# simeoncarstens/binf

Hardware: AMD Instinct MI355X
Metric: chain*leapfrog-steps/sec, 1024-d Gaussian (higher is better)
Workload: dtype f64

## Files before the change

### binf_amd/_native.py

```python
import ctypes
import linecache
import os

import torch

_HERE = os.path.dirname(os.path.abspath(__file__))
LIB_PATH = os.environ.get('BINF_LIB_OVERRIDE') or \
    os.path.join(_HERE, 'csrc', 'libbinf_hip.so')

MODE_EXACT = 0
MODE_FMA = 1
MODE_LANE_PER_CHAIN = 16
MOVE_HMC = 0
MOVE_RWMC = 1

E_ARG = -1
E_UNSUPPORTED = -2
E_ALIAS = -3


class NativeLibraryError(RuntimeError):
    """libbinf_hip.so is missing, stale or failed."""


# ... 9 lines not shown
    'binf_abi_version': (_i32, []),
    'binf_last_error': (_i32, [ctypes.c_char_p, ctypes.c_size_t]),
    'binf_hmc_sample_gauss_f64': (_i32, [_vp, _vp, _vp, _vp, _vp, _vp, _vp, _vp,
                                         _f64, _vp, _i64, _i64, _i32, _f64,
                                         _f64, _i32, _f64, _f64, _i32, _vp]),
    'binf_hmc_sample_n_gauss_f64': (_i32, [_vp, _vp, _vp, _vp, _vp, _vp, _vp,
                                           _vp, _vp, _f64, _vp, _i64, _i64,
                                           _i32, _i32, _i32, _f64, _f64, _i32,
                                           _f64, _f64, _i32, _vp]),
    'binf_hmc_gauss_waves_per_chain': (_i32, [_i64, _i64]),
    'binf_hmc_sample_gauss_big_workspace_bytes': (_i64, [_i64, _i64]),
    'binf_hmc_sample_gauss_big_f64': (_i32, [_vp, _vp, _vp, _vp, _vp, _vp, _vp, _vp,
                                             _f64, _vp, _i64, _i64, _i32, _f64,
                                             _f64, _i32, _f64, _f64, _i32, _vp,
                                             _i64, _vp]),
    'binf_hmc_sample_gauss_big_rng_f64': (_i32, [_vp, _vp, _vp, _vp, _vp, _vp, _f64, _vp,
                                                 _i64, _i64, _i32, _f64, _f64, _i32,
                                                 _f64, _f64, _i32, ctypes.c_uint64,
                                                 ctypes.c_uint64, _i64, _vp, _i64, _vp]),
    'binf_hmc_sample_n_gauss_big_workspace_bytes': (_i64, [_i64, _i64]),
    'binf_hmc_sample_n_gauss_big_f64': (_i32, [_vp, _vp, _vp, _vp, _vp, _vp, _vp, _vp, _vp,
                                               _f64, _vp, _i64, _i64, _i32, _i32, _i32, _f64,
                                               _f64, _i32, _f64, _f64, _i32, _vp, _i64, _vp]),
    'binf_hmc_sample_n_gauss_big_rng_f64': (_i32, [_vp, _vp, _vp, _vp, _vp, _vp, _vp, _f64, _vp,
                                                   _i64, _i64, _i32, _i32, _i32, _f64, _f64,
                                                   _i32, _f64, _f64, _i32, _u64, _u64, _i64,
                                                   _vp, _i64, _vp]),
    'binf_hmc_gauss_big_rng_draws_f64': (_i32, [_vp, _vp, _i64, _i64, ctypes.c_uint64,
                                                ctypes.c_uint64, _i64, _vp]),
    'binf_hmc_sample_n_gauss_rng_f64': (_i32, [_vp, _vp, _vp, _vp, _vp, _vp, _vp,
                                               _f64, _vp, _i64, _i64, _i32, _i32,
                                               _i32, _f64, _f64, _i32, _f64, _f64,
                                               _i32, ctypes.c_uint64,
                                               ctypes.c_uint64, _i64, _vp]),
    'binf_hmc_gauss_rng_draws_f64': (_i32, [_vp, _vp, _i64, _i64, _i32,
                                            ctypes.c_uint64, ctypes.c_uint64, _i64, _vp]),
    'binf_hmc_sample_poly_f64': (_i32, [_vp, _vp, _vp, _vp, _vp, _vp, _vp, _vp,
                                        _vp, _vp, _f64, _vp, _vp, _vp, _i32,
                                        _vp, _vp, _f64, _vp, _i64, _i64, _i64,
                                        _i32, _i32, _f64, _f64, _i32, _vp]),
    'binf_clipped_exp_f64': (_i32, [_vp, _vp, _i64, _vp]),
    'binf_row_sum_f64': (_i32, [_vp, _vp, _i64, _i64, _i32, _f64, _f64, _vp]),
    'binf_hmc_energy_f64': (_i32, [_vp, _vp, _vp, _i64, _i64, _vp]),
    'binf_gamma_logp_f64': (_i32, [_vp, _f64, _f64, _vp, _i64, _vp]),
    'binf_leapfrog_kick_f64': (_i32, [_vp, _vp, _f64, _vp, _i32, _i64, _i64,
                                      _i32, _vp]),
    'binf_leapfrog_drift_f64': (_i32, [_vp, _vp, _f64, _vp, _i64, _i64, _i32,
                                       _vp]),
    'binf_leapfrog_kick_drift_f64': (_i32, [_vp, _vp, _vp, _f64, _vp, _i64, _i64,
                                            _i32, _vp]),
    'binf_gauss_grad_f64': (_i32, [_vp, _vp, _f64, _f64, _i64, _i64, _vp]),
    'binf_accept_select_f64': (_i32, [_vp, _vp, _vp, _vp, _vp, _vp, _vp, _vp, _vp,
                                      _i32, _f64, _f64, _i64, _i64, _vp]),
    'binf_row_sumsq_diff_f64': (_i32, [_vp, _vp, _vp, _vp, _i64, _i64, _f64,
                                       _vp]),
    'binf_poly_forward_f64': (_i32, [_vp, _vp, _vp, _i64, _i64, _i64, _vp]),
    'binf_predictive_density_workspace_bytes': (_i64, [_i64, _i64, _i64]),
    'binf_predictive_density_f64': (_i32, [_vp, _vp, _vp, _vp, _i64, _i64, _i64, _f64, _vp, _i64, _vp]),
    'binf_gauss_err_grad_f64': (_i32, [_vp, _vp, _f64, _vp, _vp, _i64, _i64,
                                       _vp]),
    'binf_gauss_err_logp_f64': (_i32, [_vp, _vp, _f64, _vp, _vp, _i64, _i64,
                                       _vp]),
    'binf_poly_gauss_logp_f64': (_i32, [_vp, _vp, _vp, _f64, _vp, _vp, _i64,
                                        _i64, _i64, _vp]),
    'binf_poly_gauss_logp_memo_f64': (_i32, [_vp, _vp, _vp, _f64, _vp, _vp, _vp, _vp, _vp,
                                             _i64, _i64, _i64, _vp]),
    'binf_poly_gauss_grad_workspace_bytes': (_i64, [_i64, _i64, _i64]),
    'binf_poly_gauss_grad_f64': (_i32, [_vp, _vp, _vp, _f64, _vp, _vp, _vp,
                                        _i64, _i64, _i64, _i64, _vp]),
    'binf_linear_forward_f64': (_i32, [_vp, _vp, _vp, _i64, _i64, _i64, _vp]),
    'binf_linear_gauss_logp_workspace_bytes': (_i64, [_i64, _i64, _i64]),
    'binf_linear_gauss_logp_f64': (_i32, [_vp, _vp, _vp, _f64, _vp, _vp, _vp,
                                          _i64, _i64, _i64, _i64, _vp]),
    'binf_gamma_precision_update_f64': (_i32, [_vp, _vp, _f64, _vp, _i64, _vp]),
    'binf_poly_leapfrog_workspace_bytes': (_i64, [_i64, _i64, _i64]),
    'binf_poly_leapfrog_f64': (_i32, [_vp, _vp, _vp, _vp, _f64, _vp, _vp, _i64, _i64, _i64, _i64,
                                      _f64, _vp, _i32, _i32, _vp]),
    'binf_pairdist_chi2_workspace_bytes': (_i64, [_i64, _i64, _i64]),
    'binf_pairdist_gauss_logp_f64': (_i32, [_vp, _vp, _vp, _vp, _f64, _vp, _vp, _i64,
                                            _i64, _i64, _vp, _i64, _vp]),
    'binf_pairdist_gauss_logp_memo_f64': (_i32, [_vp, _vp, _vp, _vp, _f64, _vp, _vp, _vp, _vp, _vp,
                                                 _i64, _i64, _i64, _vp, _i64, _vp]),
    'binf_pairdist_forward_f64': (_i32, [_vp, _vp, _vp, _vp, _i64, _i64, _i64,
                                         _vp]),
    'binf_pairdist_gauss_grad_f64': (_i32, [_vp, _vp, _f64, _vp, _vp, _i64,
                                            _i64, _vp]),
    'binf_pairdist_leapfrog_f64': (_i32, [_vp, _vp, _vp, _f64, _vp, _i32, _f64,
                                          _f64, _i32, _f64, _vp, _i32, _i64,
                                          _i64, _i32, _vp]),
    'binf_pairdist_hmc_energy_f64': (_i32, [_vp, _vp, _vp, _vp, _vp, _f64, _vp, _f64, _f64, _i32,
                                            ctypes.POINTER(_i32), _vp, _f64, _vp, _f64,
                                            _vp, _vp, _vp, _vp, _vp, _i64, _i64, _i64, _vp, _i64, _vp]),
    'binf_pairdist_packed_targets_bytes': (_i64, [_i64]),
    'binf_pairdist_pack_targets_f64': (_i32, [_vp, _vp, _i64, _vp]),
    'binf_pairdist_tiles_workspace_bytes': (_i64, [_i64, _i64]),
    'binf_pairdist_gauss_grad_packed_f64': (_i32, [_vp, _vp, _vp, _f64, _vp, _vp, _i64,
                                                   _i64, _vp, _i64, _vp]),
    'binf_pairdist_leapfrog_packed_f64': (_i32, [_vp, _vp, _vp, _vp, _vp, _f64, _vp, _i32, _f64,
                                                 _f64, _i32, _f64, _vp, _i32, _i64,
                                                 _i64, _i32, _vp, _i64, _vp]),
    'binf_rng_uniform_f64': (_i32, [_vp, _i64, ctypes.c_uint64, ctypes.c_uint64,
                                    _i64, _vp]),
    'binf_rng_normal_f64': (_i32, [_vp, _i64, ctypes.c_uint64, ctypes.c_uint64,
                                   _i64, _vp]),
    'binf_rng_normal_zig_uniform_f64': (_i32, [_vp, _i64, _vp, _i64, ctypes.c_uint64, ctypes.c_uint64,
                                               ctypes.c_uint64, _i64, _i64, _vp]),
# ... 320 lines not shown
def metric_comoments(x, k0, s1, s2, first):
    C, D = _cd(x)
    G = _groups(s2, C, D, *_CHOL_FACTORS)
    rc = lib().binf_metric_comoments_f64(
        dptr(x, numel=C * D, name='x'), dptr(k0, numel=G * D, name='k0'),
        dptr(s1, numel=G * D, name='s1'), dptr(s2, numel=G * D * D, name='s2'),
        int(bool(first)), C, D, G, stream_handle(x.device))
    check(rc, 'binf_metric_comoments_f64')


@_launcher
def metric_factor(s1, s2, n, C, chol, work, status=None, regularise=True):
    D = s2.shape[-1]
    G = _groups(s2, int(C), D, *_CHOL_FACTORS)
    rc = lib().binf_metric_factor_f64(
        dptr(s1, numel=G * D, name='s1'), dptr(s2, numel=G * D * D, name='s2'), int(n), int(C),
        D, G, int(bool(regularise)), dptr(chol, numel=G * D * D, name='chol'),
        dptr(work, numel=G * D * D, name='work'), dptr(status, torch.int32, G, 'status'),
        stream_handle(s2.device))
    check(rc, 'binf_metric_factor_f64')


@_launcher
def gauss_grad(x, k, x0, out=None):
    C, D = _cd(x)
    if out is None:
        out = torch.empty_like(x)
    rc = lib().binf_gauss_grad_f64(dptr(x, numel=C * D, name='x'),
                                   dptr(out, numel=C * D, name='out'),
                                   float(k), float(x0), C, D,
                                   stream_handle(x.device))
    check(rc, 'binf_gauss_grad_f64')
    return out


@_launcher
def accept_select(q_prop, q_old, e_before, e_after, u, q_out, accepted,
                  n_accepted=None, dt_chain=None, adapt=False, uprate=1.05, downrate=0.95):
    C, D = _cd(q_prop)
    n = C * D
    rc = lib().binf_accept_select_f64(
        dptr(q_prop, numel=n, name='q_prop'), dptr(q_old, numel=n, name='q_old'),
        dptr(e_before, numel=C, name='e_before'),
        dptr(e_after, numel=C, name='e_after'), dptr(u, numel=C, name='u'),
        dptr(q_out, numel=n, name='q_out'),
        dptr(accepted, torch.uint8, C, 'accepted'),
        dptr(n_accepted, torch.int64, C, 'n_accepted'),
        dptr(dt_chain, numel=C, name='dt_chain'), int(bool(adapt)),
        float(uprate), float(downrate), C, D, stream_handle(q_prop.device))
    check(rc, 'binf_accept_select_f64')


@_launcher
def clipped_exp(x):
    require_device(x, 'x')
    xc = x.contiguous()
    out = torch.empty_like(xc)
    rc = lib().binf_clipped_exp_f64(dptr(xc), dptr(out), xc.numel(),
                                    stream_handle(x.device))
    check(rc, 'binf_clipped_exp_f64')
    return out


def require_device(x, what):
    if not (isinstance(x, torch.Tensor) and x.is_cuda):
        raise TypeError('%s must be a ROCm (cuda) fp64 tensor, got %s; binf_amd '
                        'evaluates on the GPU only (no CPU path)'
                        % (what, type(x).__name__ if not isinstance(x, torch.Tensor)
                           else 'a %s tensor' % x.device.type))
    return x


def _precision_args(precision, C, device):
    if isinstance(precision, torch.Tensor):
        if precision.dim() == 0:
            return float(precision), None
        p = precision.reshape(-1)
        if p.numel() != C:
            raise ValueError('precision has %d entries for %d chains'
                             % (p.numel(), C))
        return 0.0, p.contiguous()
    return float(precision), None


@_launcher
def row_sumsq_diff(x, y, scale=1.0, weights=None):
    C, D = _cd(x)
    out = torch.empty(C, dtype=torch.float64, device=x.device)
    rc = lib().binf_row_sumsq_diff_f64(dptr(x, numel=C * D, name='x'),
                                       dptr(y, numel=D, name='y'),
                                       dptr(weights, numel=D, name='weights'),
                                       dptr(out), C, D, float(scale),
                                       stream_handle(x.device))
    check(rc, 'binf_row_sumsq_diff_f64')
    return out


@_launcher
def poly_forward(coeffs, xs):
    C, K = _cd(coeffs)
    N = xs.numel()
    out = torch.empty((C, N), dtype=torch.float64, device=coeffs.device)
    rc = lib().binf_poly_forward_f64(dptr(coeffs, numel=C * K, name='coeffs'),
                                     dptr(xs, numel=N, name='xs'), dptr(out),
                                     C, K, N, stream_handle(coeffs.device))
    check(rc, 'binf_poly_forward_f64')
# ... 1129 lines not shown
```

### binf_amd/csrc/gauss_common.hpp

```cpp
#pragma once
#include "common.hpp"

namespace binf {

struct GaussNArgs {
    const double *q0;
    const double *p0;
    const double *u;
    double *q_out;
    double *samples;
    uint8_t *accepted;
    int64_t *n_accepted;
    double *e_before;
    double *e_after;
    double *dt_chain;
    double timestep;
    double k;
    double x0;
    double uprate;
    double downrate;
    int64_t C;
    int32_t D;
    int32_t nsteps;
    int32_t H;
// ... 20 lines not shown
    int LW;
    int tneed;
    bool regular;
    int64_t blocks;
};

inline GaussPlan gauss_plan(int64_t C, int64_t D)
{
    GaussPlan p;
    p.H = pairwise_tree_height(D);
    p.LW = p.H > 3 ? p.H - 3 : 0;
    p.tneed = 1;
    p.regular = true;
    int32_t len0 = -1;
    for (int g = 0; g < (1 << p.H); ++g) {
        Leaf L = pairwise_leaf((int32_t)D, p.H, g);
        int tn = (L.len + 7) / 8;
        if (tn > p.tneed) p.tneed = tn;
        if (len0 < 0) len0 = L.len;
        if (L.len != len0 || L.depth != p.H || (L.len & 7)) p.regular = false;
    }
    if (p.LW == 0) {
        const int64_t chains_per_wave = 64 >> (3 + p.H);
        const int64_t waves = (C + chains_per_wave - 1) / chains_per_wave;
        p.blocks = (waves + 3) / 4;
    } else {
        const int64_t chains_per_block = (p.LW == 3 ? 8 : 4) >> p.LW;
        p.blocks = (C + chains_per_block - 1) / chains_per_block;
    }
    return p;
}

int gauss_split_factor(int64_t C, int32_t H, bool regular, int tneed);
hipError_t launch_gauss_split(const GaussNArgs &a, int tneed, int split, bool unit, bool fma,
                              hipStream_t st);

struct LaneSum {
    double r;
    double tail;
};

template <bool REGULAR>
__device__ inline void lane_sum_add(LaneSum &s, double v, int t, int T)
{
    if (REGULAR) {
        s.r = (t == 0) ? v : s.r + v;
    } else {
        const double n = s.r + v;
        s.r = (t == 0) ? v : ((t < T) ? n : s.r);
        s.tail = (t == T) ? v : s.tail;
    }
}

template <bool REGULAR, int LW = 0>
__device__ inline double chain_sum_finish(const LaneSum &s, int T, int rem,
                                          int lane, int H, int leafdepth,
                                          double *xch = nullptr, int wib = 0)
{
    const double r = sum8_f64(s.r);
    double res = r;
    if (!REGULAR) {
        res = (T > 0) ? r : -0.0;
        const int leafbase = lane & ~7;
#pragma unroll
        for (int i = 0; i < 7; ++i) {
            const double v = shfl_f64(s.tail, leafbase + i);
            const double n = res + v;
            res = (i < rem) ? n : res;
        }
    }
    const int hin = (LW > 0) ? 3 : H;
    for (int l = 0; l < hin; ++l) {
        const double o = xor_level_f64(res, l, lane);
        const double n = res + o;
        res = (leafdepth >= H - l) ? n : res;
    }
    if (LW > 0) {
#pragma unroll
        for (int l = 3; l < 3 + LW; ++l) {
            __syncthreads();
            if (lane == 0) xch[wib] = res;
            __syncthreads();
            const double o = xch[wib ^ (1 << (l - 3))];
            const double n = res + o;
            res = (leafdepth >= H - l) ? n : res;
        }
    }
    return 0.0 + res;
}

template <int H, int N>
__device__ inline void chain_sum_finish_fixed(double (&v)[N], int lane)
{
    static_assert(H >= 0 && H <= 3, "one-wave chains: at most 8 leaves");
#pragma unroll
    for (int i = 0; i < N; ++i) v[i] = v[i] + xor1_f64(v[i]);
#pragma unroll
    for (int i = 0; i < N; ++i) v[i] = v[i] + xor2_f64(v[i]);
#pragma unroll
    for (int i = 0; i < N; ++i) v[i] = v[i] + other_quad_f64(v[i]);
#pragma unroll
    for (int l = 0; l < H; ++l) {
#pragma unroll
        for (int i = 0; i < N; ++i) v[i] = v[i] + xor_level_f64(v[i], l, lane);
    }
#pragma unroll
// ... 56 lines not shown
    r = pair_xor8_f64(r, c);
    r = sum_xor16_f64(r);
    r = sum_xor32_f64(r);
    return 0.0 + r;
}

__device__ inline double sgpr_const(unsigned long long bits)
{
    double c = __longlong_as_double((long long)bits);
    asm volatile("" : "+s"(c));
    return c;
}

__device__ inline double exp_clipped_range(double x)
{
    const double n = __builtin_rint(x * sgpr_const(0x3ff71547652b82feULL));
    double r = __builtin_fma(sgpr_const(0xbfe62e42fefa39efULL), n, x);
    r = __builtin_fma(sgpr_const(0xbc7abc9e3b39803fULL), n, r);
    double p = __builtin_fma(sgpr_const(0x3e5ade156a5dcb37ULL), r,
                             sgpr_const(0x3e928af3fca7ab0cULL));
    p = __builtin_fma(r, p, sgpr_const(0x3ec71dee623fde64ULL));
    p = __builtin_fma(r, p, sgpr_const(0x3efa01997c89e6b0ULL));
    p = __builtin_fma(r, p, sgpr_const(0x3f2a01a014761f6eULL));
    p = __builtin_fma(r, p, sgpr_const(0x3f56c16c1852b7b0ULL));
    p = __builtin_fma(r, p, sgpr_const(0x3f81111111122322ULL));
    p = __builtin_fma(r, p, sgpr_const(0x3fa55555555502a1ULL));
    p = __builtin_fma(r, p, sgpr_const(0x3fc5555555555511ULL));
    p = __builtin_fma(r, p, sgpr_const(0x3fe000000000000bULL));
    p = __builtin_fma(r, p, 1.0);
    p = __builtin_fma(r, p, 1.0);
    return __builtin_ldexp(p, (int)n);
}

template <bool BOUNDS = true>
__device__ inline bool metropolis_accept(double u, double x)
{
    if (!BOUNDS) {
        x = (x < -308.0) ? -308.0 : x;
        x = (x > 709.0) ? 709.0 : x;
        return u < exp_clipped_range(x);
    }
    const double margin = 0x1p-40;
    const double lo = (1.0 + x) - margin;
    const bool small = x >= -0.5 && x < 0.0;
    bool acc = (x >= 0.0 && u < 1.0) || (small && u < lo);
    if (!(acc || (small && u >= (1.0 + x + x * x * 0.5) + margin))) {
        x = (x < -308.0) ? -308.0 : x;
        x = (x > 709.0) ? 709.0 : x;
        acc = u < exp_clipped_range(x);
    }
    return acc;
}

__device__ inline double np_exp(double x)
{
    if (x > 709.782712893384) return __builtin_inf();
    if (x < -745.2) return 0.0;
    return exp_clipped_range(x);
}

template <bool UNIT>
__device__ inline double gauss_grad(double q, double k, double x0)
{
    return UNIT ? q : k * (q - x0);
}

template <bool FMA>
__device__ inline double kick(double p, double dt, double g)
{
    return FMA ? __builtin_fma(-dt, g, p) : p - dt * g;
}

template <bool FMA>
__device__ inline double drift(double q, double p, double dt)
{
    return FMA ? __builtin_fma(p, dt, q) : q + p * dt;
}

}
```

### binf_amd/csrc/generic.hip

```cpp
#include "rowsum.hpp"
#include "gauss_common.hpp"
#include "leapfrog_ew.hpp"

namespace binf {

enum { OP_SUM = 0, OP_SUMSQ = 1, OP_SUMSQ_SHIFT = 2, OP_SUMSQ_DIFF = 3, OP_SUMSQ_DIFF_DIV = 4 };

struct RedArgs {
    const double *x;
    const double *y;
    const double *w;
    double shift;
    int64_t D;
};

template <int OP>
struct RedElem {
    const double *row;
    const double *y;
    const double *w;
    double shift;
    __device__ inline double operator()(int i) const
    {
        const double x = row[i];
// ... 43 lines not shown
    const double *e_after;
    const double *u;
    double *q_out;
    uint8_t *accepted;
    int64_t *n_accepted;
    double *dt_chain;
    double uprate;
    double downrate;
    int64_t C;
    int64_t D;
    int32_t adapt;
    int32_t lpc;
};

template <int VEC>
__global__ void __launch_bounds__(256) accept_select_kernel(const AcceptArgs a)
{
    const int lpc = a.lpc;
    const int sub = threadIdx.x & (lpc - 1);
    const int64_t c = (int64_t)blockIdx.x * (256 / lpc) + threadIdx.x / lpc;
    if (c >= a.C) return;
    const bool acc = metropolis_accept(a.u[c], -(a.e_after[c] - a.e_before[c]));
    const double *src = (acc ? a.q_prop : a.q_old) + c * a.D;
    double *dst = a.q_out + c * a.D;
    if (dst != src) {
        for (int64_t i = (int64_t)sub * VEC; i < a.D; i += (int64_t)lpc * VEC) {
            double r[VEC];
            ew_load<VEC>(r, src, i);
            ew_store<VEC>(dst, i, r);
        }
    }
    if (sub == 0) {
        a.accepted[c] = acc ? 1 : 0;
        if (a.n_accepted && acc) a.n_accepted[c] += 1;
        if (a.adapt) {
            const double dt = a.dt_chain[c];
            a.dt_chain[c] = acc ? dt * a.uprate : dt * a.downrate;
        }
    }
}

__global__ void __launch_bounds__(256)
clipped_exp_kernel(const double *x, double *out, int64_t n)
{
    for (int64_t i = (int64_t)blockIdx.x * 256 + threadIdx.x; i < n;
         i += (int64_t)gridDim.x * 256) {
        double v = x[i];
        v = (v < -308.0) ? -308.0 : v;
        v = (v > 709.0) ? 709.0 : v;
        out[i] = exp_clipped_range(v);
    }
}

}

using namespace binf;

extern "C" int32_t binf_clipped_exp_f64(const double *x, double *out, int64_t n,
                                        void *stream)
{
    if (n < 0) return fail(BINF_E_ARG, "clipped_exp: negative size");
    if (n == 0) return 0;
    if (!x || !out) return fail(BINF_E_ARG, "clipped_exp: null buffer");
    int64_t blocks = (n + 255) / 256;
    if (blocks > 65536) blocks = 65536;
    clipped_exp_kernel<<<dim3((unsigned)blocks), 256, 0, (hipStream_t)stream>>>(x, out, n);
    hipError_t e = hipGetLastError();
    if (e != hipSuccess) return hip_fail(e, "clipped_exp launch");
    return 0;
}

extern "C" int32_t binf_row_sum_f64(const double *x, double *out, int64_t C,
                                    int64_t D, int32_t op, double shift,
                                    double scale, void *stream)
{
    if (C < 0 || D < 0) return fail(BINF_E_ARG, "row_sum: negative size");
    if (op < 0 || op > 2) return fail(BINF_E_ARG, "row_sum: unknown op %d", op);
    if (C == 0) return 0;
    if ((!x && D > 0) || !out) return fail(BINF_E_ARG, "row_sum: null buffer");
    RedArgs a;
    a.x = x; a.y = nullptr; a.w = nullptr; a.shift = shift; a.D = D;
    hipStream_t st = (hipStream_t)stream;
    switch (op) {
    case OP_SUM: return row_reduce_launch<RedMake<OP_SUM>, RedArgs>(a, C, D, scale, out, st, false, "row_sum");
    case OP_SUMSQ: return row_reduce_launch<RedMake<OP_SUMSQ>, RedArgs>(a, C, D, scale, out, st, false, "row_sum");
    default: return row_reduce_launch<RedMake<OP_SUMSQ_SHIFT>, RedArgs>(a, C, D, scale, out, st, false, "row_sum");
    }
}

extern "C" int32_t binf_hmc_energy_f64(const double *p, const double *log_prob, double *out,
                                       int64_t C, int64_t D, void *stream)
{
    if (C < 0 || D < 0) return fail(BINF_E_ARG, "hmc_energy: negative size");
    if (C == 0) return 0;
    if ((!p && D > 0) || !log_prob || !out) return fail(BINF_E_ARG, "hmc_energy: null buffer");
    RedArgs a;
    a.x = p; a.y = nullptr; a.w = nullptr; a.shift = 0.0; a.D = D;
    GaussFinish fin;
    fin.on = 2; fin.tau = 1.0; fin.tau_chain = nullptr; fin.n_data = 0.0; fin.minus = log_prob;
    return row_reduce_launch<RedMake<OP_SUMSQ>, RedArgs>(a, C, D, 0.5, out, (hipStream_t)stream, false,
                                                        "hmc_energy", &fin);
}

extern "C" int32_t binf_row_sumsq_diff_f64(const double *x, const double *y,
                                           const double *w, double *out,
                                           int64_t C, int64_t D, double scale,
                                           void *stream)
{
    if (C < 0 || D < 0) return fail(BINF_E_ARG, "row_sumsq_diff: negative size");
// ... 109 lines not shown
```

### binf_amd/csrc/hmc_gauss.hip

```cpp
#include "hmc_gauss_kernel.hpp"

namespace binf {

template <int TMAX, bool REGULAR, int LW, bool UDT = false, int HC = -1>
static hipError_t launch_n_trl(const GaussNArgs &a, bool unit, bool fma, dim3 grid,
                               hipStream_t st)
{
    constexpr int BS = (LW == 3) ? 512 : 256;
    constexpr int R = GAUSS_RNG_HBM;
    if (unit) {
        if (fma) hmc_gauss_persist_kernel<TMAX, REGULAR, true, true, LW, R, UDT, HC><<<grid, BS, 0, st>>>(a);
        else     hmc_gauss_persist_kernel<TMAX, REGULAR, true, false, LW, R, UDT, HC><<<grid, BS, 0, st>>>(a);
    } else {
        if (fma) hmc_gauss_persist_kernel<TMAX, REGULAR, false, true, LW, R, UDT, HC><<<grid, BS, 0, st>>>(a);
        else     hmc_gauss_persist_kernel<TMAX, REGULAR, false, false, LW, R, UDT, HC><<<grid, BS, 0, st>>>(a);
    }
    return hipGetLastError();
}

static bool gauss_uniform_dt(const GaussNArgs &a)
{
    return a.dt_chain == nullptr && a.n_adapt == 0;
}

template <int TMAX, int HC>
static hipError_t launch_n_th(const GaussNArgs &a, bool unit, bool fma, dim3 grid,
                              hipStream_t st)
{
    if (gauss_uniform_dt(a))
        return launch_n_trl<TMAX, true, 0, true, HC>(a, unit, fma, grid, st);
    return launch_n_trl<TMAX, true, 0, false, HC>(a, unit, fma, grid, st);
}

template <int TMAX>
static hipError_t launch_n_t(const GaussNArgs &a, bool regular, bool unit, bool fma,
                             dim3 grid, hipStream_t st)
{
    if (!regular)
        return launch_n_trl<TMAX, false, 0>(a, unit, fma, grid, st);
    if (a.H == 0) return launch_n_th<TMAX, 0>(a, unit, fma, grid, st);
    if constexpr (TMAX >= 12) {
        if (a.H == 1) return launch_n_th<TMAX, 1>(a, unit, fma, grid, st);
        if (a.H == 2) return launch_n_th<TMAX, 2>(a, unit, fma, grid, st);
        if (a.H == 3) return launch_n_th<TMAX, 3>(a, unit, fma, grid, st);
    }
    return hipErrorNotSupported;
}

template <int LW>
static hipError_t launch_n_wide(const GaussNArgs &a, bool regular, bool unit, bool fma,
                                dim3 grid, hipStream_t st)
{
    return regular ? launch_n_trl<16, true, LW>(a, unit, fma, grid, st)
                   : launch_n_trl<16, false, LW>(a, unit, fma, grid, st);
}

}

using namespace binf;

extern "C" int32_t binf_hmc_sample_n_gauss_f64(
    const double *q0, const double *p0, const double *u, double *q_out,
    double *samples, uint8_t *accepted, int64_t *n_accepted, double *e_before,
    double *e_after, double timestep, double *dt_chain, int64_t C, int64_t D,
    int32_t nsteps, int32_t n, int32_t thin, double k, double x0,
    int32_t n_adapt, double uprate, double downrate, int32_t mode, void *stream)
{
    if (C < 0 || D < 1 || nsteps < 1 || n < 1 || thin < 1 || n_adapt < 0)
        return fail(BINF_E_ARG, "hmc_sample_gauss: need C>=0, D>=1, nsteps>=1, n>=1, thin>=1, n_adapt>=0");
    if (mode != BINF_MODE_EXACT && mode != BINF_MODE_FMA)
        return fail(BINF_E_ARG, "hmc_sample_gauss: unknown mode %d", mode);
    if (C == 0) return 0;
    if (!q0 || !p0 || !u || !q_out)
        return fail(BINF_E_ARG, "hmc_sample_gauss: null buffer");
    if (n_adapt > 0 && !dt_chain)
        return fail(BINF_E_ARG, "hmc_sample_gauss: adaption needs dt_chain");
    if (D > 8192)
        return fail(BINF_E_UNSUPPORTED, "hmc_sample_gauss: D=%lld > 8192 not covered by the fused kernel", (long long)D);
    const GaussPlan plan = gauss_plan(C, D);
    const int32_t H = plan.H;
    if (H > 6)
// ... 68 lines not shown
```

### binf_amd/csrc/hmc_gauss_kernel.hpp

```cpp
#pragma once
#include "gauss_common.hpp"
#include "xoshiro.hpp"

namespace binf {

enum { GAUSS_RNG_HBM = 0, GAUSS_RNG_FUSED = 1, GAUSS_RNG_DUMP = 2 };

constexpr int gauss_wpb(int LW, int RNG) { return (LW == 3 || RNG != GAUSS_RNG_HBM) ? 8 : 4; }

constexpr int GAUSS_STEP_UNROLL = 4;
constexpr int gauss_step_unroll(int TMAX, bool REGULAR, bool UNIT, bool FMA, int LW, int RNG)
{
    if (!REGULAR || LW != 0 || !UNIT) return 1;
    if ((TMAX == 12 && !FMA) || (TMAX == 4 && RNG == GAUSS_RNG_FUSED)) return 1;
    return GAUSS_STEP_UNROLL;
}

constexpr int GAUSS_PRIO_WINDOW = 4;
constexpr bool gauss_wave_priority(int LW, int RNG, int HC)
{
    return LW == 0 && RNG == GAUSS_RNG_HBM && HC == 3;
}

__device__ __forceinline__ void gauss_set_priority(int prio)
{
    switch (prio & 3) {
    case 0: __builtin_amdgcn_s_setprio(0); break;
    case 1: __builtin_amdgcn_s_setprio(1); break;
    case 2: __builtin_amdgcn_s_setprio(2); break;
    default: __builtin_amdgcn_s_setprio(3); break;
    }
}

template <int TMAX, bool REGULAR, bool UNIT, bool FMA, int LW, int RNG = GAUSS_RNG_HBM, bool UDT = false,
          int HC = -1>
__global__ void __launch_bounds__(64 * gauss_wpb(LW, RNG))
hmc_gauss_persist_kernel(const GaussNArgs a)
{
    static_assert(HC < 0 || (REGULAR && LW == 0), "compile-time tree height: regular one-wave chains only");
    constexpr bool FIXED = HC >= 0;
    constexpr int HF = FIXED ? HC : 0;
    constexpr bool SHARED = HC == 3;
    constexpr bool EARLY = FIXED && UNIT && !SHARED;
    constexpr int WPB = gauss_wpb(LW, RNG);
    constexpr int WPC = 1 << LW;
    __shared__ double xch[WPB];
    __shared__ double ubc[WPB];
    constexpr int GS = (TMAX % 8 == 0) ? 8 : ((TMAX % 4 == 0) ? 4 : TMAX);
    constexpr int NG = TMAX / GS;
    constexpr int USTEP = gauss_step_unroll(TMAX, REGULAR, UNIT, FMA, LW, RNG);
    constexpr bool PRIO = gauss_wave_priority(LW, RNG, HC);
    __shared__ double stash[RNG == GAUSS_RNG_DUMP ? 1 : WPB][RNG == GAUSS_RNG_DUMP ? 1 : TMAX][64];
    __shared__ double zx[RNG == GAUSS_RNG_HBM ? 1 : XZIG_C + 1];
    if (RNG != GAUSS_RNG_HBM) {
        xzig_load_table(zx, threadIdx.x, WPB * 64);
        __syncthreads();
    }

    const int lane = threadIdx.x & 63;
    const int wib = threadIdx.x >> 6;
    const int64_t wave = (int64_t)blockIdx.x * WPB + wib;
    const int H = FIXED ? HC : a.H;
    const int lg = (LW > 0) ? 6 : 3 + H;
    const int slot = lane & ((1 << lg) - 1);
    const int j = slot & 7;
    const int wchain = wib & (WPC - 1);
    const int grp = (LW > 0) ? ((wchain << 3) | (lane >> 3)) : (slot >> 3);
    const bool writer = (LW > 0) ? (wchain == 0 && lane == 0) : (slot == 0);

    int off, n, leafdepth, canonical;
    if (REGULAR) {
        n = 8 * TMAX;
        off = grp * n;
        leafdepth = H;
        canonical = 1;
    } else {
        const Leaf L = pairwise_leaf(a.D, H, grp);
        off = L.off;
        n = L.len;
        leafdepth = L.depth;
        canonical = L.canonical;
    }
    const int T = (n >= 8) ? (n >> 3) : 0;
    const int rem = (n >= 8) ? (n & 7) : n;

    const int64_t raw = (LW > 0) ? (int64_t)blockIdx.x * (WPB / WPC) + (wib >> LW)
                                 : (wave << (6 - lg)) + (lane >> lg);
    const bool cvalid = raw < a.C;
    const int64_t chain = cvalid ? raw : a.C - 1;
    const int64_t CD = a.C * (int64_t)a.D;
    const int64_t base = chain * (int64_t)a.D + off + j;

    double dt = (UDT || !a.dt_chain) ? a.timestep : a.dt_chain[chain];
    double uu = 0.0;
    if (RNG == GAUSS_RNG_HBM) uu = a.u[chain];
// ... 46 lines not shown
            for (int t = 0; t < TMAX; ++t) stash[wib][t][lane] = q[t];
        }

        const bool more = s + 1 < a.n;
        const double *pc = a.p0 + (int64_t)s * CD + base;
        const double *pn = more ? pc + CD : pc;
        double un = 0.0;
        if (RNG == GAUSS_RNG_HBM) un = a.u[(int64_t)(more ? s + 1 : s) * a.C + chain];

        LaneSum spb = {0.0, 0.0}, sqa = {0.0, 0.0}, spa = {0.0, 0.0};
        double Spb = 0.0;
#pragma unroll
        for (int g = 0; g < NG; ++g) {
            double(&cur)[GS] = (RNG == GAUSS_RNG_HBM && (g & 1)) ? pb : pa;
            double(&nxt)[GS] = (RNG == GAUSS_RNG_HBM && (g & 1)) ? pa : pb;
            if (RNG != GAUSS_RNG_HBM) {
                unsigned want = 0;
#pragma unroll
                for (int i = 0; i < GS; ++i)
                    if (REGULAR || (8 * (g * GS + i) + j < n)) want |= 1u << i;
                xzig_normals<GS>(cur, want, gen, zx);
                if (RNG == GAUSS_RNG_DUMP) {
                    if (cvalid && canonical) {
                        double *go = a.p_dump + (int64_t)s * CD + base;
#pragma unroll
                        for (int i = 0; i < GS; ++i)
                            if (want & (1u << i)) go[8 * (g * GS + i)] = cur[i];
                    }
                    continue;
                }
            } else if (g + 1 < NG) {
#pragma unroll
                for (int i = 0; i < GS; ++i) {
                    const int t = (g + 1) * GS + i;
                    const bool m = REGULAR || (8 * t + j < n);
                    nxt[i] = m ? pc[8 * t] : 0.0;
                }
            } else {
#pragma unroll
                for (int i = 0; i < GS; ++i) {
                    const bool m = REGULAR || (8 * i + j < n);
                    nxt[i] = m ? pn[8 * i] : 0.0;
                }
            }
            (void)nxt;
#pragma unroll
            for (int i = 0; i < GS; ++i)
                asm volatile("" : "+v"(cur[i]), "+v"(q[g * GS + i]));
            if (s == 0) {
#pragma unroll
                for (int i = 0; i < GS; ++i) {
                    const int t = g * GS + i;
                    const double d = UNIT ? q[t] : q[t] - a.x0;
                    lane_sum_add<REGULAR>(s0, d * d, t, T);
                }
                if (FIXED && !SHARED && g == NG - 1) {
                    double v[1] = {s0.r};
                    chain_sum_finish_fixed<HF, 1>(v, lane);
                    Sq_state = v[0];
                }
            }
#pragma unroll
            for (int i = 0; i < GS; ++i)
                lane_sum_add<REGULAR>(spb, cur[i] * cur[i], g * GS + i, T);
            __builtin_amdgcn_sched_barrier(0);
            if (EARLY && g == NG - 1) {
                double v[1] = {spb.r};
                chain_sum_finish_fixed<HF, 1>(v, lane);
                Spb = v[0];
            }
#pragma unroll
            for (int i = 0; i < GS; ++i) {
                const int t = g * GS + i;
                cur[i] = kick<FMA>(cur[i], hdt, gauss_grad<UNIT>(q[t], a.k, a.x0));
            }
            if (EARLY && g == NG - 1) asm volatile("" : "+v"(Spb));
            if (USTEP == 1) {
                for (int l = 0; l < a.nsteps - 1; ++l) {
#pragma unroll
                    for (int i = 0; i < GS; ++i) {
                        const int t = g * GS + i;
                        q[t] = drift<FMA>(q[t], cur[i], dt);
                        cur[i] = kick<FMA>(cur[i], dt, gauss_grad<UNIT>(q[t], a.k, a.x0));
                    }
                }
            } else {
                const auto step = [&]() {
#pragma unroll
                    for (int i = 0; i < GS; ++i) {
                        const int t = g * GS + i;
                        q[t] = drift<FMA>(q[t], cur[i], dt);
                        cur[i] = kick<FMA>(cur[i], dt, gauss_grad<UNIT>(q[t], a.k, a.x0));
                    }
                };
                static_assert((USTEP & (USTEP - 1)) == 0, "the remainder below goes by the bits of its count");
                const int nl = a.nsteps > 1 ? a.nsteps - 1 : 0;
#pragma unroll 1
                for (int m = nl / USTEP; m > 0; --m) {
#pragma unroll
                    for (int k = 0; k < USTEP; ++k) step();
                }
#pragma unroll
                for (int b = USTEP >> 1; b > 0; b >>= 1) {
                    if (nl & b) {
#pragma unroll
                        for (int k = 0; k < b; ++k) step();
                    }
                }
            }
#pragma unroll
            for (int i = 0; i < GS; ++i) {
                const int t = g * GS + i;
                q[t] = drift<FMA>(q[t], cur[i], dt);
                cur[i] = kick<FMA>(cur[i], hdt, gauss_grad<UNIT>(q[t], a.k, a.x0));
            }
#pragma unroll
            for (int i = 0; i < GS; ++i) {
                const int t = g * GS + i;
                const double d = UNIT ? q[t] : q[t] - a.x0;
                lane_sum_add<REGULAR>(sqa, d * d, t, T);
                lane_sum_add<REGULAR>(spa, cur[i] * cur[i], t, T);
            }
            if (EARLY && g == NG - 1)
                asm volatile("" : "+v"(sqa.r), "+v"(spa.r));
            else
                asm volatile("" : "+v"(sqa.r), "+v"(spa.r), "+v"(spb.r));
            __builtin_amdgcn_sched_barrier(0);
        }
        if (RNG != GAUSS_RNG_HBM) {
            const double ud = xo_uniform53(gen);
            if (LW == 0) {
                uu = shfl_f64(ud, lane & ~((1 << lg) - 1));
            } else {
                if (wchain == 0 && lane == 0) ubc[wib] = ud;
                __syncthreads();
                uu = ubc[wib & ~(WPC - 1)];
                __syncthreads();
            }
            if (RNG == GAUSS_RNG_DUMP) {
                if (cvalid && writer) a.u_dump[(int64_t)s * a.C + chain] = uu;
                continue;
            }
        }
        if (RNG == GAUSS_RNG_HBM && (NG & 1)) {
#pragma unroll
            for (int i = 0; i < GS; ++i) pa[i] = pb[i];
        }
        double Sqa, Spa;
        if (SHARED) {
            const double r = chain_sums_shared(sqa.r, spa.r, spb.r, s0.r, s == 0);
            Sqa = lane_value_f64<0>(r);
            Spa = lane_value_f64<4>(r);
            Spb = lane_value_f64<8>(r);
            if (s == 0) Sq_state = lane_value_f64<12>(r);
        } else if (FIXED) {
            if (EARLY) {
                double v[2] = {sqa.r, spa.r};
                chain_sum_finish_fixed<HF, 2>(v, lane);
                Sqa = v[0];
                Spa = v[1];
            } else {
                double v[3] = {spb.r, sqa.r, spa.r};
                chain_sum_finish_fixed<HF, 3>(v, lane);
                Spb = v[0];
                Sqa = v[1];
                Spa = v[2];
            }
        } else {
            if (s == 0)
                Sq_state = chain_sum_finish<REGULAR, LW>(s0, T, rem, lane, H, leafdepth, xch, wib);
            Spb = chain_sum_finish<REGULAR, LW>(spb, T, rem, lane, H, leafdepth, xch, wib);
            Sqa = chain_sum_finish<REGULAR, LW>(sqa, T, rem, lane, H, leafdepth, xch, wib);
            Spa = chain_sum_finish<REGULAR, LW>(spa, T, rem, lane, H, leafdepth, xch, wib);
        }
        const double Eb = -(c_lp * Sq_state) + 0.5 * Spb;
        const double Ea = -(c_lp * Sqa) + 0.5 * Spa;

        const bool acc = metropolis_accept<SHARED>(uu, -(Ea - Eb));

        if (!UDT && s < a.n_adapt)
            dt = acc ? dt * a.uprate : dt * a.downrate;
        if (cvalid && writer) {
            const int64_t o = (int64_t)s * a.C + chain;
            if (a.accepted) a.accepted[o] = acc ? 1 : 0;
            if (a.e_before) a.e_before[o] = Eb;
            if (a.e_after) a.e_after[o] = Ea;
        }
        if (acc) {
            Sq_state = Sqa;
            nacc += 1;
        } else {
            if (stash_lds) {
#pragma unroll
                for (int t = 0; t < TMAX; ++t) q[t] = stash[wib][t][lane];
            } else {
#pragma unroll
                for (int t = 0; t < TMAX; ++t) q[t] = prev[base + 8 * t];
            }
            __builtin_amdgcn_s_waitcnt(0);
        }
        if (a.samples && --rec_wait == 0) {
            rec_wait = a.thin;
            if (cvalid && canonical) {
                double *go = rec + base;
#pragma unroll
                for (int t = 0; t < TMAX; ++t)
                    if (REGULAR || (8 * t + j < n)) go[8 * t] = q[t];
            }
            prev = rec;
            rec += CD;
        }
        if (RNG == GAUSS_RNG_HBM) uu = un;
    }
    if (RNG == GAUSS_RNG_DUMP) return;
    if (PRIO) __builtin_amdgcn_s_setprio(0);

    if (cvalid && writer) {
        if (a.n_accepted) a.n_accepted[chain] += nacc;
        if (!UDT && a.n_adapt > 0 && a.dt_chain) a.dt_chain[chain] = dt;
    }
    if (cvalid && canonical) {
        double *go = a.q_out + base;
#pragma unroll
        for (int t = 0; t < TMAX; ++t)
            if (REGULAR || (8 * t + j < n)) go[8 * t] = q[t];
    }
}


}
```

### include/binf_hip.h

```cpp
#ifndef BINF_HIP_H
#define BINF_HIP_H

#include <stddef.h>
#include <stdint.h>

#ifdef __cplusplus
extern "C" {
#endif

#define BINF_ABI_VERSION 7

#define BINF_E_ARG        (-1)
#define BINF_E_UNSUPPORTED (-2)
#define BINF_E_ALIAS      (-3)

#define BINF_MODE_EXACT 0
#define BINF_MODE_FMA   1
#define BINF_MODE_LANE_PER_CHAIN 16

int32_t binf_abi_version(void);

int32_t binf_last_error(char *buf, size_t n);

int32_t binf_hmc_sample_gauss_f64(const double *q0, const double *p0,
// ... 71 lines not shown

int32_t binf_hmc_sample_n_gauss_rng_f64(const double *q0, double *q_out,
                                        double *samples, uint8_t *accepted,
                                        int64_t *n_accepted, double *e_before,
                                        double *e_after, double timestep,
                                        double *dt_chain, int64_t C, int64_t D,
                                        int32_t nsteps, int32_t n, int32_t thin,
                                        double k, double x0, int32_t n_adapt,
                                        double uprate, double downrate,
                                        int32_t mode, uint64_t seed,
                                        uint64_t offset, int64_t chain_offset,
                                        void *stream);

int32_t binf_hmc_gauss_rng_draws_f64(double *p0_out, double *u_out, int64_t C,
                                     int64_t D, int32_t n, uint64_t seed,
                                     uint64_t offset, int64_t chain_offset,
                                     void *stream);


#define BINF_ROW_SUM 0
#define BINF_ROW_SUMSQ 1
#define BINF_ROW_SUMSQ_SHIFT 2
int32_t binf_row_sum_f64(const double *x, double *out, int64_t C, int64_t D,
                         int32_t op, double shift, double scale, void *stream);

int32_t binf_hmc_energy_f64(const double *p, const double *log_prob, double *out,
                            int64_t C, int64_t D, void *stream);

int32_t binf_leapfrog_kick_f64(double *p, const double *grad, double timestep,
                               const double *dt_chain, int32_t half, int64_t C,
                               int64_t D, int32_t mode, void *stream);

int32_t binf_leapfrog_drift_f64(double *q, const double *p, double timestep,
                                const double *dt_chain, int64_t C, int64_t D,
                                int32_t mode, void *stream);

int32_t binf_leapfrog_kick_drift_f64(double *q, double *p, const double *grad,
                                     double timestep, const double *dt_chain,
                                     int64_t C, int64_t D, int32_t mode,
                                     void *stream);

int32_t binf_gauss_grad_f64(const double *x, double *out, double k, double x0,
                            int64_t C, int64_t D, void *stream);

int32_t binf_clipped_exp_f64(const double *x, double *out, int64_t n, void *stream);

int32_t binf_accept_select_f64(const double *q_prop, const double *q_old,
                               const double *e_before, const double *e_after,
                               const double *u, double *q_out, uint8_t *accepted,
                               int64_t *n_accepted, double *dt_chain,
                               int32_t adapt, double uprate,
                               double downrate, int64_t C, int64_t D,
                               void *stream);

int32_t binf_row_sumsq_diff_f64(const double *x, const double *y, const double *w,
                                double *out, int64_t C, int64_t D, double scale,
                                void *stream);


int32_t binf_poly_forward_f64(const double *coeffs, const double *xs, double *out,
                              int64_t C, int64_t K, int64_t N, void *stream);

int32_t binf_gauss_err_grad_f64(const double *mock, const double *ys,
                                double precision, const double *precision_chain,
                                double *out, int64_t C, int64_t N, void *stream);

int32_t binf_gauss_err_logp_f64(const double *mock, const double *ys,
                                double precision, const double *precision_chain,
                                double *out, int64_t C, int64_t N, void *stream);

int32_t binf_poly_gauss_logp_f64(const double *coeffs, const double *xs,
                                 const double *ys, double precision,
                                 const double *precision_chain, double *out,
                                 int64_t C, int64_t K, int64_t N, void *stream);

int32_t binf_poly_gauss_logp_memo_f64(const double *coeffs, const double *xs,
                                      const double *ys, double precision,
                                      const double *precision_chain, double *out,
                                      double *memo_coeffs, double *memo_chi2,
                                      uint8_t *memo_state, int64_t C, int64_t K, int64_t N,
                                      void *stream);

int64_t binf_poly_gauss_grad_workspace_bytes(int64_t C, int64_t K, int64_t N);
int32_t binf_poly_gauss_grad_f64(const double *coeffs, const double *design,
                                 const double *ys, double precision,
                                 const double *precision_chain, double *out,
                                 void *workspace, int64_t workspace_bytes,
                                 int64_t C, int64_t K, int64_t N, void *stream);

int64_t binf_poly_leapfrog_workspace_bytes(int64_t C, int64_t K, int64_t N);
int32_t binf_poly_leapfrog_f64(double *q, double *p, const double *design,
                               const double *ys, double precision,
                               const double *precision_chain, void *workspace,
                               int64_t workspace_bytes, int64_t C, int64_t K,
                               int64_t N, double timestep, const double *dt_chain,
                               int32_t nsteps, int32_t mode, void *stream);


int32_t binf_linear_forward_f64(const double *coeffs, const double *design, double *out,
                                int64_t C, int64_t K, int64_t N, void *stream);

int64_t binf_linear_gauss_logp_workspace_bytes(int64_t C, int64_t K, int64_t N);
int32_t binf_linear_gauss_logp_f64(const double *coeffs, const double *design,
                                   const double *ys, double precision,
                                   const double *precision_chain, double *out,
                                   void *workspace, int64_t workspace_bytes,
// ... 398 lines not shown
```

Baseline: 5.404 billion.

## Fuse energy sums into FMAs with certified accept and exact fallback recompute

For the shared-tree Gaussian HMC kernel with no energy outputs requested, the per-chain energy sums are accumulated with fused multiply-adds instead of the exact pairwise-ordered adds. A rounding-error-bounded Metropolis decision is then made. If any lane in the wave is undecided, the trajectory is recomputed with exact sums to reproduce the bitwise-exact accept. This trims arithmetic from the hot sum loop. It adds a rare, expensive re-simulation path, extra register pressure, and new template instantiations. A standalone accept_decide kernel and API are also exposed.

```diff
diff --git a/binf_amd/_native.py b/binf_amd/_native.py
--- a/binf_amd/_native.py
+++ b/binf_amd/_native.py
@@ -85,6 +85,7 @@
     'binf_gauss_grad_f64': (_i32, [_vp, _vp, _f64, _f64, _i64, _i64, _vp]),
     'binf_accept_select_f64': (_i32, [_vp, _vp, _vp, _vp, _vp, _vp, _vp, _vp, _vp,
                                       _i32, _f64, _f64, _i64, _i64, _vp]),
+    'binf_accept_decide_f64': (_i32, [_vp, _vp, _vp, _vp, _i64, _vp]),
     'binf_row_sumsq_diff_f64': (_i32, [_vp, _vp, _vp, _vp, _i64, _i64, _f64,
                                        _vp]),
     'binf_poly_forward_f64': (_i32, [_vp, _vp, _vp, _i64, _i64, _i64, _vp]),
@@ -511,6 +512,19 @@
 
 
 @_launcher
+def accept_decide(u, x, delta):
+    require_device(u, 'u')
+    n = u.numel()
+    out = torch.empty(n, dtype=torch.int32, device=u.device)
+    rc = lib().binf_accept_decide_f64(dptr(u, numel=n, name='u'), dptr(x, numel=n, name='x'),
+                                      dptr(delta, numel=n, name='delta'),
+                                      dptr(out, torch.int32, n, 'out'), n,
+                                      stream_handle(u.device))
+    check(rc, 'binf_accept_decide_f64')
+    return out
+
+
+@_launcher
 def clipped_exp(x):
     require_device(x, 'x')
     xc = x.contiguous()
diff --git a/binf_amd/csrc/gauss_common.hpp b/binf_amd/csrc/gauss_common.hpp
--- a/binf_amd/csrc/gauss_common.hpp
+++ b/binf_amd/csrc/gauss_common.hpp
@@ -96,6 +96,11 @@
     }
 }
 
+__device__ inline void lane_sum_fused(LaneSum &s, double x, int t)
+{
+    s.r = (t == 0) ? x * x : __builtin_fma(x, x, s.r);
+}
+
 template <bool REGULAR, int LW = 0>
 __device__ inline double chain_sum_finish(const LaneSum &s, int T, int rem,
                                           int lane, int H, int leafdepth,
@@ -258,6 +263,29 @@
     return acc;
 }
 
+enum { GAUSS_REJECT = 0, GAUSS_ACCEPT = 1, GAUSS_UNDECIDED = 2 };
+
+__device__ inline int accept_decide(double u, double x, double delta)
+{
+    const double margin = 0x1p-40;
+    const bool ok = (unsigned long long)__double_as_longlong(u) < 0x3ff0000000000000ULL &&
+                    (unsigned long long)__double_as_longlong(delta) <= 0x3ea0000000000000ULL &&
+                    __builtin_fabs(x) < __builtin_inf();
+    const double xl = x - delta, xh = x + delta;
+    const bool inb = xl >= -0.5;
+    bool acc = inb && u < (1.0 + xl) - margin;
+    bool rej = inb && xh < 0.0 && u >= (1.0 + xh + xh * xh * 0.5) + margin;
+    if (ok && !(acc || rej)) {
+        double c = (x < -308.0) ? -308.0 : x;
+        c = (c > 709.0) ? 709.0 : c;
+        const double y = exp_clipped_range(c);
+        const double w = (delta + delta) * y;
+        acc = u < (y - w) - margin;
+        rej = u >= (y + w) + margin;
+    }
+    return (!ok || !(acc || rej)) ? GAUSS_UNDECIDED : (acc ? GAUSS_ACCEPT : GAUSS_REJECT);
+}
+
 __device__ inline double np_exp(double x)
 {
     if (x > 709.782712893384) return __builtin_inf();
diff --git a/binf_amd/csrc/generic.hip b/binf_amd/csrc/generic.hip
--- a/binf_amd/csrc/generic.hip
+++ b/binf_amd/csrc/generic.hip
@@ -119,9 +119,31 @@
     }
 }
 
+__global__ void __launch_bounds__(256)
+accept_decide_kernel(const double *u, const double *x, const double *delta, int32_t *out, int64_t n)
+{
+    for (int64_t i = (int64_t)blockIdx.x * 256 + threadIdx.x; i < n;
+         i += (int64_t)gridDim.x * 256)
+        out[i] = accept_decide(u[i], x[i], delta[i]);
+}
+
 }
 
 using namespace binf;
+
+extern "C" int32_t binf_accept_decide_f64(const double *u, const double *x, const double *delta,
+                                          int32_t *out, int64_t n, void *stream)
+{
+    if (n < 0) return fail(BINF_E_ARG, "accept_decide: negative size");
+    if (n == 0) return 0;
+    if (!u || !x || !delta || !out) return fail(BINF_E_ARG, "accept_decide: null buffer");
+    int64_t blocks = (n + 255) / 256;
+    if (blocks > 65536) blocks = 65536;
+    accept_decide_kernel<<<dim3((unsigned)blocks), 256, 0, (hipStream_t)stream>>>(u, x, delta, out, n);
+    hipError_t e = hipGetLastError();
+    if (e != hipSuccess) return hip_fail(e, "accept_decide launch");
+    return 0;
+}
 
 extern "C" int32_t binf_clipped_exp_f64(const double *x, double *out, int64_t n,
                                         void *stream)
diff --git a/binf_amd/csrc/hmc_gauss.hip b/binf_amd/csrc/hmc_gauss.hip
--- a/binf_amd/csrc/hmc_gauss.hip
+++ b/binf_amd/csrc/hmc_gauss.hip
@@ -2,18 +2,20 @@
 
 namespace binf {
 
-template <int TMAX, bool REGULAR, int LW, bool UDT = false, int HC = -1>
+template <int TMAX, bool REGULAR, int LW, bool UDT = false, int HC = -1, bool FS = false>
 static hipError_t launch_n_trl(const GaussNArgs &a, bool unit, bool fma, dim3 grid,
                                hipStream_t st)
 {
     constexpr int BS = (LW == 3) ? 512 : 256;
     constexpr int R = GAUSS_RNG_HBM;
+    constexpr bool FU = FS && gauss_fastsum_built(TMAX, HC, true);
+    constexpr bool FN = FS && gauss_fastsum_built(TMAX, HC, false);
     if (unit) {
-        if (fma) hmc_gauss_persist_kernel<TMAX, REGULAR, true, true, LW, R, UDT, HC><<<grid, BS, 0, st>>>(a);
-        else     hmc_gauss_persist_kernel<TMAX, REGULAR, true, false, LW, R, UDT, HC><<<grid, BS, 0, st>>>(a);
+        if (fma) hmc_gauss_persist_kernel<TMAX, REGULAR, true, true, LW, R, UDT, HC, FU><<<grid, BS, 0, st>>>(a);
+        else     hmc_gauss_persist_kernel<TMAX, REGULAR, true, false, LW, R, UDT, HC, FU><<<grid, BS, 0, st>>>(a);
     } else {
-        if (fma) hmc_gauss_persist_kernel<TMAX, REGULAR, false, true, LW, R, UDT, HC><<<grid, BS, 0, st>>>(a);
-        else     hmc_gauss_persist_kernel<TMAX, REGULAR, false, false, LW, R, UDT, HC><<<grid, BS, 0, st>>>(a);
+        if (fma) hmc_gauss_persist_kernel<TMAX, REGULAR, false, true, LW, R, UDT, HC, FN><<<grid, BS, 0, st>>>(a);
+        else     hmc_gauss_persist_kernel<TMAX, REGULAR, false, false, LW, R, UDT, HC, FN><<<grid, BS, 0, st>>>(a);
     }
     return hipGetLastError();
 }
@@ -27,6 +29,13 @@
 static hipError_t launch_n_th(const GaussNArgs &a, bool unit, bool fma, dim3 grid,
                               hipStream_t st)
 {
+    if constexpr (HC == 3) {
+        if (a.e_before == nullptr && a.e_after == nullptr) {
+            if (gauss_uniform_dt(a))
+                return launch_n_trl<TMAX, true, 0, true, HC, true>(a, unit, fma, grid, st);
+            return launch_n_trl<TMAX, true, 0, false, HC, true>(a, unit, fma, grid, st);
+        }
+    }
     if (gauss_uniform_dt(a))
         return launch_n_trl<TMAX, true, 0, true, HC>(a, unit, fma, grid, st);
     return launch_n_trl<TMAX, true, 0, false, HC>(a, unit, fma, grid, st);
diff --git a/binf_amd/csrc/hmc_gauss_kernel.hpp b/binf_amd/csrc/hmc_gauss_kernel.hpp
--- a/binf_amd/csrc/hmc_gauss_kernel.hpp
+++ b/binf_amd/csrc/hmc_gauss_kernel.hpp
@@ -32,8 +32,60 @@
     }
 }
 
+constexpr int GAUSS_REDO_GS = 2;
+template <int TMAX, int GS, bool UNIT, bool FMA>
+__device__ inline bool gauss_exact_accept(const GaussNArgs &a, const double *qs, const double (*qs_lds)[64],
+                                          int lane, const double *pc, double dt, double hdt, double c_lp,
+                                          double u)
+{
+    LaneSum s0 = {0.0, 0.0}, spb = {0.0, 0.0}, sqa = {0.0, 0.0}, spa = {0.0, 0.0};
+#pragma unroll 1
+    for (int g = 0; g < TMAX / GS; ++g) {
+        double qq[GS], pp[GS];
+#pragma unroll
+        for (int i = 0; i < GS; ++i) {
+            const int t = g * GS + i;
+            qq[i] = qs_lds ? qs_lds[t][lane] : qs[8 * t];
+            pp[i] = pc[8 * t];
+        }
+#pragma unroll
+        for (int i = 0; i < GS; ++i) {
+            const int t = g * GS + i;
+            const double d = UNIT ? qq[i] : qq[i] - a.x0;
+            lane_sum_add<true>(s0, d * d, t, TMAX);
+            lane_sum_add<true>(spb, pp[i] * pp[i], t, TMAX);
+        }
+#pragma unroll
+        for (int i = 0; i < GS; ++i)
+            pp[i] = kick<FMA>(pp[i], hdt, gauss_grad<UNIT>(qq[i], a.k, a.x0));
+#pragma unroll 1
+        for (int l = 0; l < a.nsteps - 1; ++l) {
+#pragma unroll
+            for (int i = 0; i < GS; ++i) {
+                qq[i] = drift<FMA>(qq[i], pp[i], dt);
+                pp[i] = kick<FMA>(pp[i], dt, gauss_grad<UNIT>(qq[i], a.k, a.x0));
+            }
+        }
+#pragma unroll
+        for (int i = 0; i < GS; ++i) {
+            const int t = g * GS + i;
+            qq[i] = drift<FMA>(qq[i], pp[i], dt);
+            pp[i] = kick<FMA>(pp[i], hdt, gauss_grad<UNIT>(qq[i], a.k, a.x0));
+            const double d = UNIT ? qq[i] : qq[i] - a.x0;
+            lane_sum_add<true>(sqa, d * d, t, TMAX);
+            lane_sum_add<true>(spa, pp[i] * pp[i], t, TMAX);
+        }
+    }
+    const double r = chain_sums_shared(sqa.r, spa.r, spb.r, s0.r, true);
+    const double Eb = -(c_lp * lane_value_f64<12>(r)) + 0.5 * lane_value_f64<8>(r);
+    const double Ea = -(c_lp * lane_value_f64<0>(r)) + 0.5 * lane_value_f64<4>(r);
+    return metropolis_accept<true>(u, -(Ea - Eb));
+}
+
+constexpr bool gauss_fastsum_built(int TMAX, int HC, bool UNIT) { return HC == 3 && (TMAX == 16 || !UNIT); }
+
 template <int TMAX, bool REGULAR, bool UNIT, bool FMA, int LW, int RNG = GAUSS_RNG_HBM, bool UDT = false,
-          int HC = -1>
+          int HC = -1, bool FASTSUM = false>
 __global__ void __launch_bounds__(64 * gauss_wpb(LW, RNG))
 hmc_gauss_persist_kernel(const GaussNArgs a)
 {
@@ -41,6 +93,7 @@
     constexpr bool FIXED = HC >= 0;
     constexpr int HF = FIXED ? HC : 0;
     constexpr bool SHARED = HC == 3;
+    static_assert(!FASTSUM || (SHARED && RNG == GAUSS_RNG_HBM), "fused sums: the shared-tree kernels, draws from HBM");
     constexpr bool EARLY = FIXED && UNIT && !SHARED;
     constexpr int WPB = gauss_wpb(LW, RNG);
     constexpr int WPC = 1 << LW;
@@ -193,7 +246,8 @@
                 for (int i = 0; i < GS; ++i) {
                     const int t = g * GS + i;
                     const double d = UNIT ? q[t] : q[t] - a.x0;
-                    lane_sum_add<REGULAR>(s0, d * d, t, T);
+                    if (FASTSUM) lane_sum_fused(s0, d, t);
+                    else lane_sum_add<REGULAR>(s0, d * d, t, T);
                 }
                 if (FIXED && !SHARED && g == NG - 1) {
                     double v[1] = {s0.r};
@@ -202,8 +256,10 @@
                 }
             }
 #pragma unroll
-            for (int i = 0; i < GS; ++i)
-                lane_sum_add<REGULAR>(spb, cur[i] * cur[i], g * GS + i, T);
+            for (int i = 0; i < GS; ++i) {
+                if (FASTSUM) lane_sum_fused(spb, cur[i], g * GS + i);
+                else lane_sum_add<REGULAR>(spb, cur[i] * cur[i], g * GS + i, T);
+            }
             __builtin_amdgcn_sched_barrier(0);
             if (EARLY && g == NG - 1) {
                 double v[1] = {spb.r};
@@ -259,8 +315,13 @@
             for (int i = 0; i < GS; ++i) {
                 const int t = g * GS + i;
                 const double d = UNIT ? q[t] : q[t] - a.x0;
-                lane_sum_add<REGULAR>(sqa, d * d, t, T);
-                lane_sum_add<REGULAR>(spa, cur[i] * cur[i], t, T);
+                if (FASTSUM) {
+                    lane_sum_fused(sqa, d, t);
+                    lane_sum_fused(spa, cur[i], t);
+                } else {
+                    lane_sum_add<REGULAR>(sqa, d * d, t, T);
+                    lane_sum_add<REGULAR>(spa, cur[i] * cur[i], t, T);
+                }
             }
             if (EARLY && g == NG - 1)
                 asm volatile("" : "+v"(sqa.r), "+v"(spa.r));
@@ -317,7 +378,18 @@
         const double Eb = -(c_lp * Sq_state) + 0.5 * Spb;
         const double Ea = -(c_lp * Sqa) + 0.5 * Spa;
 
-        const bool acc = metropolis_accept<SHARED>(uu, -(Ea - Eb));
+        bool acc;
+        if (FASTSUM) {
+            const int dec = accept_decide(uu, -(Ea - Eb), 0x1p-46 * (Eb + Ea));
+            acc = dec == GAUSS_ACCEPT;
+            if (__builtin_amdgcn_ballot_w64(dec == GAUSS_UNDECIDED || !(c_lp < 0.0)) != 0) {
+                acc = gauss_exact_accept<TMAX, GAUSS_REDO_GS, UNIT, FMA>(
+                    a, prev + base, stash_lds ? stash[wib] : nullptr, lane, pc, dt, hdt, c_lp, uu);
+                __builtin_amdgcn_s_waitcnt(0);
+            }
+        } else {
+            acc = metropolis_accept<SHARED>(uu, -(Ea - Eb));
+        }
 
         if (!UDT && s < a.n_adapt)
             dt = acc ? dt * a.uprate : dt * a.downrate;
diff --git a/include/binf_hip.h b/include/binf_hip.h
--- a/include/binf_hip.h
+++ b/include/binf_hip.h
@@ -147,6 +147,12 @@
                                int32_t adapt, double uprate,
                                double downrate, int64_t C, int64_t D,
                                void *stream);
+
+#define BINF_ACCEPT_NO 0
+#define BINF_ACCEPT_YES 1
+#define BINF_ACCEPT_UNDECIDED 2
+int32_t binf_accept_decide_f64(const double *u, const double *x, const double *delta,
+                               int32_t *out, int64_t n, void *stream);
 
 int32_t binf_row_sumsq_diff_f64(const double *x, const double *y, const double *w,
                                 double *out, int64_t C, int64_t D, double scale,
```

Result: faster. 5.471 billion (median of 6 runs) (+1.2%).
